# NOC-OI/ship-track-estimators

Hardware: AMD Instinct MI355X
Metric: UKF+URTSS track-steps/sec (dim=4, 500-step tracks) (higher is better)
Workload: dtype f64

## Files before the change

### ship-track-estimators_amd/csrc/ste_kernels.hip

```cpp
#include <hip/hip_runtime.h>

#include <algorithm>
#include <cstddef>
#include <cstdint>
#include <cstdio>
#include <cstring>
#include <type_traits>
#include <vector>

#include "../../include/ste.h"
#include "ste_err.h"
#include "ste_ukf.h"

namespace ste {

__shared__ int g_sched_word[2];
__device__ __forceinline__ int sched_k0() { return *(volatile int*)&g_sched_word[0]; }

template <bool kWarm>
__device__ __forceinline__ int sigma_fan(const double (&x)[4], const double (&P)[4][4], double scale,
                                         double (&sig)[9][4], EigBasis& basis);

__device__ __forceinline__ int sigma_fan(const double (&x)[4], const double (&P)[4][4], double scale,
                                         double (&sig)[9][4]) {
// ... 519 lines not shown
__device__ __forceinline__ int lane_update(const Mats& p, double (&x)[4], double (&P)[10], const double (&zin)[4],
                                           const double* noise, size_t nrow, size_t B, size_t t, UpdLik* lik = nullptr,
                                           const double* Rt = nullptr) {
    if (kFastUpd) {
        double z[4];
        STE_UNROLL
        for (int c = 0; c < 4; ++c) z[c] = zin[c];
        double r00 = p.R[0], r01 = p.R[1], r11 = p.R[5];
        if constexpr (kTrackR) {
            if (Rt) {
                r00 = Rt[(size_t)tix(0, 0) * B];
                r01 = Rt[(size_t)tix(0, 1) * B];
                r11 = Rt[(size_t)tix(1, 1) * B];
            }
        }
        int st = 0;
        if (kRobust) st = robust_rescale_sel2(p, x, P, z, r00, r01, r11);
        if (noise) {
            STE_UNROLL
            for (int c = 0; c < 4; ++c) z[c] += noise[(nrow * 4 + c) * B + t];
        }
        lane_update_sel2<kLik>(r00, r01, r11, x, P, z, lik);
        return st;
    } else {
        double Pf[4][4];
        STE_UNROLL
        for (int r = 0; r < 4; ++r) {
            STE_UNROLL
            for (int c = 0; c < 4; ++c) Pf[r][c] = P[tix(r, c)];
        }
        const int st = ukf_update<kLik, kTrackR>(p, x, Pf, zin, noise, nrow, B, t, lik, Rt);
        STE_UNROLL
        for (int r = 0; r < 4; ++r) {
            STE_UNROLL
            for (int c = r; c < 4; ++c) P[tix(r, c)] = Pf[r][c];
        }
        return st;
    }
}

__device__ __forceinline__ void store_hist(const KParams& p, size_t row, size_t B, size_t t, const double (&x)[4],
                                           const double (&P)[10]) {
    STE_UNROLL
    for (int c = 0; c < 4; ++c) st_stream(&p.fwd_mean[(row * 4 + c) * B + t], x[c]);
    store_cov_p(p.fwd_cov, (p.flags & STE_FLAG_PACKED_COV) != 0, row, B, t, P);
}

enum { kLikOff = 0, kLikHist = 1, kLikOnly = 2 };
struct LikParams {
    double* loglik;
    int32_t* dof;
    int32_t* nupd;
    double* nis;
};

template <bool kGains, bool kFastUpd, bool kRobust, bool kSched, int kLik = kLikOff, bool kTrackNoise = false>
__device__ __forceinline__ void forward_tile_l1(const KParams& p, const size_t t, const LikParams* lk = nullptr,
                                                const NoiseParams* nz = nullptr) {
    static_assert(kLik != kLikOnly || (!kGains && !kSched), "the likelihood-only pass writes no histories and no work rows");
    const size_t B = (size_t)p.ld;
    if (t >= (size_t)p.B) return;
    const bool cont = (p.flags & kFlagContinue) != 0;
    const int ns = (p.nsteps ? p.nsteps[t] - p.k0 : p.Nmax);
    if (cont && ns <= 0) return;

    double x[4], P[10];
    STE_UNROLL
    for (int c = 0; c < 4; ++c) x[c] = p.x0[c * B + t];
    if (cont && (p.flags & STE_FLAG_PACKED_COV)) {
        load_cov_p(p.P0, true, 0, B, t, P);
    } else {
        double Pf[4][4];
        if (p.flags & STE_FLAG_SHARED_P0) {
            STE_UNROLL
            for (int r = 0; r < 4; ++r) {
                STE_UNROLL
                for (int c = 0; c < 4; ++c) Pf[r][c] = p.P0[r * 4 + c];
            }
        } else {
            load_mat(p.P0, 0, B, t, Pf);
        }
        STE_UNROLL
        for (int r = 0; r < 4; ++r) {
            STE_UNROLL
            for (int c = r; c < 4; ++c) P[tix(r, c)] = 0.5 * (Pf[r][c] + Pf[c][r]);
        }
    }
    if (kLik != kLikOnly) store_hist(p, 0, B, t, x, P);

    int st = cont ? (__hip_atomic_load(&p.status[t], __ATOMIC_RELAXED, __HIP_MEMORY_SCOPE_AGENT) & ~STE_STATUS_NAN) : 0;
    const bool initial_update = !(p.flags & STE_FLAG_NO_INITIAL_UPDATE);
    const bool noise_mode = p.noise_pred || p.noise_upd || p.noise_rts;
    bool flagged = false;
    double* first_bad = (kGains && p.rts_work) ? p.first_bad + t : nullptr;
    if (first_bad) {
        if (cont)
            flagged = __hip_atomic_load(first_bad, __ATOMIC_RELAXED, __HIP_MEMORY_SCOPE_AGENT) != kNeverBad;
        else
            *first_bad = kNeverBad;
    }
    TrigReg tk;
    trig_reg_init(tk);
    double Qv[10];
    STE_UNROLL
    for (int r = 0; r < 4; ++r) {
        STE_UNROLL
        for (int c = r; c < 4; ++c) Qv[tix(r, c)] = in_vgpr(p.m.Q[r * 4 + c]);
    }
    const double* Rt = nullptr;
    if constexpr (kTrackNoise) {
        if (nz->Q) {
            STE_UNROLL
            for (int e = 0; e < 10; ++e) Qv[e] = nz->Q[(size_t)e * B + t];
        }
        if (nz->R) Rt = nz->R + t;
    }
    double V[4][4];
    if (kGains && initial_update && ns > 0) {
        double xc[4], Pc[10];
        STE_UNROLL
        for (int c = 0; c < 4; ++c) xc[c] = x[c];
        STE_UNROLL
        for (int e = 0; e < 10; ++e) Pc[e] = P[e];
        st |= lane_predict<true, kSched>(p.m, xc, Pc, V, false, p.dt[t], p.sog_rate[t], p.cog_rate[t], nullptr, p.noise_rts, 0, B, t,
                                         p.rts_work, true, noise_mode, flagged, first_bad, tk, Qv);
    }
    double lik_sum = 0.0;
    int lik_dof = 0, lik_nupd = 0;
    if (initial_update) {
        double z0[4];
        load_vec(p.z, 0, B, t, z0);
        if constexpr (kLik != kLikOff) {
            UpdLik u;
            st |= lane_update<kFastUpd, kRobust, true, kTrackNoise>(p.m, x, P, z0, p.noise_upd, 0, B, t, &u, Rt);
            lik_sum += update_loglik(u);
            lik_dof += u.rank;
            lik_nupd += 1;
            if (lk->nis) st_stream(&lk->nis[t], u.nis);
        } else {
            st |= lane_update<kFastUpd, kRobust, false, kTrackNoise>(p.m, x, P, z0, p.noise_upd, 0, B, t, nullptr, Rt);
        }
    } else if (kLik != kLikOff && lk->nis) {
        st_stream(&lk->nis[t], __builtin_nan(""));
    }

    double dt_n = 0.0, sr_n = 0.0, cr_n = 0.0;
    int ui_n = -1;
    if (ns > 0) {
        dt_n = p.dt[t];
        sr_n = p.sog_rate[t];
        cr_n = p.cog_rate[t];
        ui_n = p.upd_idx[t];
    }
    for (int k = 0; k < p.Nmax; ++k) {
        const bool live = k < ns;
        if (!__any(live)) break;
        if (live) {
            const double dt = dt_n, sr = sr_n, cr = cr_n;
            const int ui = ui_n;
            const bool ui_ok = ui < p.Tmax;
            const bool upd = ui >= 0 && ui_ok;
            double zk[4];
            load_vec(p.z, (size_t)(upd ? ui : 0), B, t, zk);
            {
                const size_t o = (size_t)(k + 1 < ns ? k + 1 : k) * B + t;
                dt_n = p.dt[o];
                sr_n = p.sog_rate[o];
                cr_n = p.cog_rate[o];
                ui_n = p.upd_idx[o];
            }
            double* work = (kGains && !(k == 0 && initial_update)) ? p.rts_work : nullptr;
            const bool warm = (k & (kColdEvery - 1)) != 0;
            st |= lane_predict<kGains, kSched>(p.m, x, P, V, warm, dt, sr, cr, p.noise_pred, p.noise_rts, (size_t)k, B, t, work,
                                               upd || noise_mode, noise_mode, flagged, first_bad, tk, Qv);
            if constexpr (kLik != kLikOff) {
                UpdLik u;
                u.nis = __builtin_nan("");
                if (upd) {
                    st |= lane_update<kFastUpd, kRobust, true, kTrackNoise>(p.m, x, P, zk, p.noise_upd, (size_t)k + 1, B, t, &u, Rt);
                    lik_sum += update_loglik(u);
                    lik_dof += u.rank;
                    lik_nupd += 1;
                }
                if (lk->nis) st_stream(&lk->nis[((size_t)k + 1) * B + t], u.nis);
            } else {
                if (upd) st |= lane_update<kFastUpd, kRobust, false, kTrackNoise>(p.m, x, P, zk, p.noise_upd, (size_t)k + 1, B, t, nullptr, Rt);
            }
            if (!ui_ok) st |= STE_STATUS_BAD_INDEX;
            if (kLik != kLikOnly) store_hist(p, (size_t)k + 1, B, t, x, P);
        }
    }
    double chk = 0.0;
    STE_UNROLL
    for (int c = 0; c < 4; ++c) chk += x[c] * 0.0;
    STE_UNROLL
    for (int e = 0; e < 10; ++e) chk += P[e] * 0.0;
    if (!(chk == 0.0)) st |= STE_STATUS_NAN;
    p.status[t] = st;
    if constexpr (kLik != kLikOff) {
        lk->loglik[t] = lik_sum;
        if (lk->dof) lk->dof[t] = lik_dof;
        if (lk->nupd) lk->nupd[t] = lik_nupd;
    }
}

template <bool kGains, bool kFastUpd, bool kRobust = false>
__global__ __launch_bounds__(64) __attribute__((amdgpu_waves_per_eu(1, 1))) void ukf_forward_l1(const KParams p) {
    forward_tile_l1<kGains, kFastUpd, kRobust, false>(p, (size_t)blockIdx.x * 64 + threadIdx.x);
}

template <bool kGains, bool kFastUpd, bool kRobust, int kLik>
__global__ __launch_bounds__(64) __attribute__((amdgpu_waves_per_eu(1, 1))) void ukf_forward_lik(const KParams p, const LikParams l) {
    forward_tile_l1<kGains, kFastUpd, kRobust, false, kLik>(p, (size_t)blockIdx.x * 64 + threadIdx.x, &l);
}

template <bool kGains, bool kFastUpd, bool kRobust, int kLik>
__global__ __launch_bounds__(64) __attribute__((amdgpu_waves_per_eu(1, 1))) void ukf_forward_tn(const KParams p, const LikParams l,
                                                                                                 const NoiseParams nz) {
    forward_tile_l1<kGains, kFastUpd, kRobust, false, kLik, true>(p, (size_t)blockIdx.x * 64 + threadIdx.x, &l, &nz);
}

struct SchedItem {
    int kp;
    int tile;
    int prog;
    int meta;
};
struct SchedParams {
    const KParams* kps;
    const SchedItem* items;
    int nrounds, nwaves;
    int* progress;
    int* window_done;
    int* error;
    unsigned long long timeout_ticks;
    int* started;
};

template <bool kGains, bool kFastUpd, bool kRobust>
__global__ __launch_bounds__(64) __attribute__((amdgpu_waves_per_eu(1, 1))) void ukf_forward_sched(const SchedParams sp) {
    typedef const KParams __attribute__((address_space(4))) ConstKParams;
    if (sp.started && threadIdx.x == 0) __hip_atomic_fetch_add(sp.started, 1, __ATOMIC_RELAXED, __HIP_MEMORY_SCOPE_AGENT);
    for (int r = 0; r < sp.nrounds; ++r) {
        const SchedItem* ip = sp.items + ((size_t)r * sp.nwaves + blockIdx.x);
        const int kp = __builtin_amdgcn_readfirstlane(ip->kp);
        if (kp < 0) continue;
        const int tile_word = __builtin_amdgcn_readfirstlane(ip->tile), prog = __builtin_amdgcn_readfirstlane(ip->prog);
        const int tile = tile_word & 0xffffff, publish = (tile_word >> 24) & 0xff;
        const int meta = __builtin_amdgcn_readfirstlane(ip->meta);
        const int slice = meta & 0xff;
        if (meta < 0 && (__hip_atomic_load(sp.error, __ATOMIC_RELAXED, __HIP_MEMORY_SCOPE_AGENT) != 0 ||
                         !sched_wait(sp.progress + prog, slice, sp.timeout_ticks))) {
            if (threadIdx.x == 0) __hip_atomic_store(sp.error, 1, __ATOMIC_RELAXED, __HIP_MEMORY_SCOPE_AGENT);
            return;
        }
        const KParams& p = *(const KParams*)(ConstKParams*)(uintptr_t)(sp.kps + kp);
        if (threadIdx.x == 0) *(volatile int*)&g_sched_word[0] = p.k0;
        forward_tile_l1<kGains, kFastUpd, kRobust, true>(p, (size_t)tile * 64 + threadIdx.x);
        if (meta & 0x40000000) {
            asm volatile("s_waitcnt vmcnt(0)" ::: "memory");
            __builtin_amdgcn_fence(__ATOMIC_RELEASE, "agent");
            asm volatile("s_waitcnt vmcnt(0)" ::: "memory");
            if (threadIdx.x == 0) {
                __hip_atomic_store(sp.progress + prog, publish, __ATOMIC_RELAXED, __HIP_MEMORY_SCOPE_AGENT);
                if (meta & 0x100)
                    __hip_atomic_fetch_add(sp.window_done + ((meta >> 9) & 0x1fffff), 1, __ATOMIC_RELAXED, __HIP_MEMORY_SCOPE_AGENT);
            }
        }
    }
}

__global__ __launch_bounds__(256) void sched_upload(uint4* __restrict__ dst, const uint4* __restrict__ src, size_t ncopy, size_t nzero) {
    const size_t stride = (size_t)gridDim.x * blockDim.x;
    for (size_t i = (size_t)blockIdx.x * blockDim.x + threadIdx.x; i < ncopy + nzero; i += stride)
        dst[i] = i < ncopy ? src[i] : make_uint4(0, 0, 0, 0);
}

__global__ __launch_bounds__(64) void sched_gate(const int* counter, int need, int* error, unsigned long long timeout_ticks) {
    if (!sched_wait(counter, need, timeout_ticks) && threadIdx.x == 0 && error)
        __hip_atomic_store(error, 2, __ATOMIC_RELAXED, __HIP_MEMORY_SCOPE_AGENT);
}


template <bool kTrackNoise>
__global__ __launch_bounds__(64) void urtss_backward_l1(const KParams p, const NoiseParams nz) {
    const size_t B = (size_t)p.ld;
    const size_t t = (size_t)blockIdx.x * 64 + threadIdx.x;
    if (t >= (size_t)p.B) return;
    auto track_Q = [&](int r, int c) -> double {
        if constexpr (kTrackNoise)
            return nz.Q[(size_t)tix(r, c) * B + t];
        else
            return p.m.Q[r * 4 + c];
    };
    const int ns = p.nsteps ? p.nsteps[t] : p.Nmax;
    const double* srp = p.sog_rate_rts ? p.sog_rate_rts : p.sog_rate;
    const double* crp = p.cog_rate_rts ? p.cog_rate_rts : p.cog_rate;

    double xs[4], Ps[4][4];
    load_vec(p.fwd_mean, (size_t)ns, B, t, xs);
    const bool packed = (p.flags & STE_FLAG_PACKED_COV) != 0;
    load_cov_m(p.fwd_cov, packed, (size_t)ns, B, t, Ps);
    store_vec(p.sm_mean, (size_t)ns, B, t, xs);
    store_cov_m(p.sm_cov, packed, (size_t)ns, B, t, Ps);
    store_pos(p, (size_t)ns, B, t, xs);

// ... 1004 lines not shown
```

### ship-track-estimators_amd/csrc/ste_math.h

```cpp
#pragma once
#include <hip/hip_runtime.h>

namespace ste {

constexpr double kEarthRadius = 6378.137;
constexpr double kDeg2Rad = 0.017453292519943295;
constexpr double kRad2Deg = 57.29577951308232;
constexpr double kPinvRcond = 1e-15;
constexpr int kMaxSweeps = 12;
constexpr double kRotTol2 = 4.930380657631324e-32;

#define STE_UNROLL _Pragma("unroll")

struct Mats {
    double fan_scale, w0, wi;
    double H[16], Q[16], R[16];
    double chi_alpha;
    int robust_iters;
};

__device__ __forceinline__ double floored_mod360(double a) {
    if (__builtin_expect(!(fabs(a) < 1e15), 0)) {
        double r = fmod(a, 360.0);
        if (r != 0.0) {
            if (r < 0.0) r += 360.0;
        } else {
            r = 0.0;
        }
        return r;
    }
    double q = floor(a * 2.7777777777777778e-03);
    double r = fma(-q, 360.0, a);
    if (r < 0.0) {
        q -= 1.0;
        r = fma(-q, 360.0, a);
    } else if (r >= 360.0) {
        q += 1.0;
        r = fma(-q, 360.0, a);
        if (r < 0.0) r = 360.0;
    }
    return r;
}
__device__ __forceinline__ double floored_mod(double a, double b) {
    (void)b;
    return floored_mod360(a);
}

__device__ __forceinline__ double wrap180(double y) { return floored_mod(y + 180.0, 360.0) - 180.0; }

__device__ __forceinline__ double rsqrt_fast(double x) {
    const double y = __builtin_amdgcn_rsq(x);
    const double e = fma(-(x * y), y, 1.0);
    return fma(y * e, fma(0.375, e, 0.5), y);
}


__device__ __forceinline__ void sincos_kernel(double r, double& s, double& c) {
    const double z = r * r;
    double ps = fma(z, 1.58969099521155010221e-10, -2.50507602534068634195e-08);
    ps = fma(z, ps, 2.75573137070700676789e-06);
    ps = fma(z, ps, -1.98412698298579493134e-04);
    ps = fma(z, ps, 8.33333333332248946124e-03);
    ps = fma(z, ps, -1.66666666666666324348e-01);
    s = fma(z * r, ps, r);
    double pc = fma(z, -1.13596475577881948265e-11, 2.08757232129817482790e-09);
    pc = fma(z, pc, -2.75573143513906633035e-07);
    pc = fma(z, pc, 2.48015872894767294178e-05);
    pc = fma(z, pc, -1.38888888888741095749e-03);
    pc = fma(z, pc, 4.16666666666666019037e-02);
    c = fma(z * z, pc, fma(-0.5, z, 1.0));
}

__device__ __forceinline__ void sincos_fast(double x, double& s, double& c) {
    if (__builtin_expect(!(fabs(x) < 1048576.0), 0)) {
        sincos(x, &s, &c);
        return;
    }
    const double n = rint(x * 0.63661977236758134308);
    double r = fma(-n, 1.57079632679489655800e+00, x);
    r = fma(-n, 6.12323399573676603587e-17, r);
    r = fma(-n, -1.49738490485916983405e-33, r);
    double sk, ck;
    sincos_kernel(r, sk, ck);
    const int q = (int)n;
    const double sv = (q & 1) ? ck : sk;
    const double cv = (q & 1) ? sk : ck;
    s = (q & 2) ? -sv : sv;
    c = ((q + 1) & 2) ? -cv : cv;
}

__device__ __forceinline__ double atan_small(double q) {
    const double z = q * q, w = z * z;
    double s1 = fma(w, 1.62858201153657823623e-02, 4.97687799461593236017e-02);
    s1 = fma(w, s1, 6.66107313738753120669e-02);
    s1 = fma(w, s1, 9.09088713343650656196e-02);
    s1 = fma(w, s1, 1.42857142725034663711e-01);
    s1 = fma(w, s1, 3.33333333333329318027e-01);
    double s2 = fma(w, -3.65315727442169155270e-02, -5.83357013379057348645e-02);
    s2 = fma(w, s2, -7.69187620504482999495e-02);
    s2 = fma(w, s2, -1.11111104054623557880e-01);
    s2 = fma(w, s2, -1.99999999998764832476e-01);
    return fma(-q, fma(z, s1, w * s2), q);
}

__device__ __forceinline__ double div_pos(double a, double b) {
    double r = __builtin_amdgcn_rcp(b);
    r = fma(fma(-b, r, 1.0), r, r);
    const double q = a * r;
    return fma(fma(-b, q, a), r, q);
}

__device__ __forceinline__ double div_earth_radius(double a) {
    constexpr double kInvR = 1.0 / kEarthRadius;
    const double q = a * kInvR;
    return fma(fma(-q, kEarthRadius, a), kInvR, q);
}

__device__ __forceinline__ double atan2_fast(double a, double b) {
    if (__builtin_expect(b > 1e-300 && fabs(a) <= 0.4375 * b, 1)) return atan_small(div_pos(a, b));
    return atan2(a, b);
}

__device__ __forceinline__ double asin_small(double x) {
    const double t = x * x;
    double pn = fma(t, 3.47933107596021167570e-05, 7.91534994289814532176e-04);
    pn = fma(t, pn, -4.00555345006794114027e-02);
    pn = fma(t, pn, 2.01212532134862925881e-01);
    pn = fma(t, pn, -3.25565818622400915405e-01);
    pn = fma(t, pn, 1.66666666666666657415e-01);
    pn *= t;
    double qd = fma(t, 7.70381505559019352791e-02, -6.88283971605453293030e-01);
    qd = fma(t, qd, 2.02094576023350569471e+00);
    qd = fma(t, qd, -2.40339491173441421878e+00);
    qd = fma(t, qd, 1.0);
    return fma(x, div_pos(pn, qd), x);
}

__device__ __forceinline__ void geodetic_finish(double lon_r, double lat_r, double sp, double cp, double sa, double ca,
                                                double sd, double cd, double& lon_out, double& lat_out) {
    const double a = sd * sa;
    const double sdca = sd * ca;
    const double b = fma(cp, cd, -(sp * sdca));
    const double sl = fma(sp, cd, cp * sdca);
    lon_out = (lon_r + atan2_fast(a, b)) * kRad2Deg;
    const double h2 = fma(a, a, b * b);
    const double cl = h2 * rsqrt_fast(h2);
    const double xs = fma(sl, cp, -(cl * sp));
    double lat2;
    if (__builtin_expect(fabs(xs) <= 0.5 && h2 > 1e-300 && cd > 0.0, 1)) {
        lat2 = lat_r + asin_small(xs);
    } else {
        lat2 = asin(sl);
    }
    lat_out = lat2 * kRad2Deg;
}

__device__ __forceinline__ void sincos_delta(double d, double& s, double& c) {
    if (__builtin_expect(fabs(d) <= 0.78539816339744828, 1)) {
        sincos_kernel(d, s, c);
    } else {
        sincos_fast(d, s, c);
    }
}

struct TrigLit {
    static constexpr double s1 = 1.58969099521155010221e-10, s2 = -2.50507602534068634195e-08, s3 = 2.75573137070700676789e-06,
                            s4 = -1.98412698298579493134e-04, s5 = 8.33333333332248946124e-03, s6 = -1.66666666666666324348e-01;
    static constexpr double c1 = -1.13596475577881948265e-11, c2 = 2.08757232129817482790e-09, c3 = -2.75573143513906633035e-07,
                            c4 = 2.48015872894767294178e-05, c5 = -1.38888888888741095749e-03, c6 = 4.16666666666666019037e-02;
};
struct TrigReg {
    double s1, s2, s3, s4, s5, s6, c1, c2, c3, c4, c5, c6;
};
__device__ __forceinline__ double in_vgpr(double v) {
    asm volatile("" : "+v"(v));
    return v;
}
__device__ __forceinline__ void trig_reg_init(TrigLit&) {}
__device__ __forceinline__ void trig_reg_init(TrigReg& k) {
    k.s1 = in_vgpr(TrigLit::s1);
    k.s2 = in_vgpr(TrigLit::s2);
    k.s3 = in_vgpr(TrigLit::s3);
    k.s4 = in_vgpr(TrigLit::s4);
    k.s5 = in_vgpr(TrigLit::s5);
    k.s6 = in_vgpr(TrigLit::s6);
    k.c1 = in_vgpr(TrigLit::c1);
    k.c2 = in_vgpr(TrigLit::c2);
    k.c3 = in_vgpr(TrigLit::c3);
    k.c4 = in_vgpr(TrigLit::c4);
    k.c5 = in_vgpr(TrigLit::c5);
    k.c6 = in_vgpr(TrigLit::c6);
}

template <int N, class K = TrigLit>
__device__ __forceinline__ void sincos_kernel_n(const double (&r)[N], double (&s)[N], double (&c)[N], const K& k = K()) {
#pragma clang fp contract(off)
    double z[N], ps[N], pc[N];
    STE_UNROLL
    for (int i = 0; i < N; ++i) z[i] = r[i] * r[i];
    STE_UNROLL
    for (int i = 0; i < N; ++i) ps[i] = fma(z[i], k.s1, k.s2);
    STE_UNROLL
    for (int i = 0; i < N; ++i) ps[i] = fma(z[i], ps[i], k.s3);
    STE_UNROLL
    for (int i = 0; i < N; ++i) ps[i] = fma(z[i], ps[i], k.s4);
    STE_UNROLL
    for (int i = 0; i < N; ++i) ps[i] = fma(z[i], ps[i], k.s5);
    STE_UNROLL
    for (int i = 0; i < N; ++i) ps[i] = fma(z[i], ps[i], k.s6);
    STE_UNROLL
    for (int i = 0; i < N; ++i) s[i] = fma(z[i] * r[i], ps[i], r[i]);
    STE_UNROLL
    for (int i = 0; i < N; ++i) pc[i] = fma(z[i], k.c1, k.c2);
    STE_UNROLL
    for (int i = 0; i < N; ++i) pc[i] = fma(z[i], pc[i], k.c3);
    STE_UNROLL
    for (int i = 0; i < N; ++i) pc[i] = fma(z[i], pc[i], k.c4);
    STE_UNROLL
    for (int i = 0; i < N; ++i) pc[i] = fma(z[i], pc[i], k.c5);
    STE_UNROLL
    for (int i = 0; i < N; ++i) pc[i] = fma(z[i], pc[i], k.c6);
    STE_UNROLL
    for (int i = 0; i < N; ++i) c[i] = fma(z[i] * z[i], pc[i], fma(-0.5, z[i], 1.0));
}

template <int N, class K = TrigLit>
__device__ __forceinline__ void sincos_fast_n(const double (&x)[N], double (&s)[N], double (&c)[N], bool& ok,
                                              const K& k = K()) {
#pragma clang fp contract(off)
    double n[N], r[N], sk[N], ck[N];
    double x_max = fabs(x[0]);
    STE_UNROLL
    for (int i = 1; i < N; ++i) x_max = fmax(x_max, fabs(x[i]));
    ok = ok && (x_max < 1048576.0);
    STE_UNROLL
    for (int i = 0; i < N; ++i) n[i] = rint(x[i] * 0.63661977236758134308);
    STE_UNROLL
    for (int i = 0; i < N; ++i) r[i] = fma(-n[i], 1.57079632679489655800e+00, x[i]);
    STE_UNROLL
    for (int i = 0; i < N; ++i) r[i] = fma(-n[i], 6.12323399573676603587e-17, r[i]);
    STE_UNROLL
    for (int i = 0; i < N; ++i) r[i] = fma(-n[i], -1.49738490485916983405e-33, r[i]);
    sincos_kernel_n<N, K>(r, sk, ck, k);
    STE_UNROLL
    for (int i = 0; i < N; ++i) {
        const int q = (int)n[i];
        const double sv = (q & 1) ? ck[i] : sk[i];
        const double cv = (q & 1) ? sk[i] : ck[i];
        s[i] = (q & 2) ? -sv : sv;
        c[i] = ((q + 1) & 2) ? -cv : cv;
    }
}

template <int N, class K = TrigLit>
__device__ __forceinline__ void sincos_delta_n(const double (&d)[N], double (&s)[N], double (&c)[N], bool& ok,
                                               const K& k = K()) {
#pragma clang fp contract(off)
    double d_max = fabs(d[0]);
    STE_UNROLL
    for (int i = 1; i < N; ++i) d_max = fmax(d_max, fabs(d[i]));
    ok = ok && (d_max <= 0.78539816339744828);
    sincos_kernel_n<N, K>(d, s, c, k);
}

struct GeoLit {
    static constexpr double t0 = 1.62858201153657823623e-02, t1 = 4.97687799461593236017e-02, t2 = 6.66107313738753120669e-02,
                            t3 = 9.09088713343650656196e-02, t4 = 1.42857142725034663711e-01, t5 = 3.33333333333329318027e-01,
                            u0 = -3.65315727442169155270e-02, u1 = -5.83357013379057348645e-02, u2 = -7.69187620504482999495e-02,
                            u3 = -1.11111104054623557880e-01, u4 = -1.99999999998764832476e-01;
    static constexpr double p0 = 3.47933107596021167570e-05, p1 = 7.91534994289814532176e-04, p2 = -4.00555345006794114027e-02,
                            p3 = 2.01212532134862925881e-01, p4 = -3.25565818622400915405e-01, p5 = 1.66666666666666657415e-01,
                            q0 = 7.70381505559019352791e-02, q1 = -6.88283971605453293030e-01, q2 = 2.02094576023350569471e+00,
                            q3 = -2.40339491173441421878e+00;
};
struct GeoReg {
    double t0, t1, t2, t3, t4, t5, u0, u1, u2, u3, u4;
    static constexpr double p0 = GeoLit::p0, p1 = GeoLit::p1, p2 = GeoLit::p2, p3 = GeoLit::p3, p4 = GeoLit::p4, p5 = GeoLit::p5,
                            q0 = GeoLit::q0, q1 = GeoLit::q1, q2 = GeoLit::q2, q3 = GeoLit::q3;
};
__device__ __forceinline__ void geo_reg_init(GeoLit&) {}
__device__ __forceinline__ void geo_reg_init(GeoReg& k) {
    k.t0 = in_vgpr(GeoLit::t0);
    k.t1 = in_vgpr(GeoLit::t1);
    k.t2 = in_vgpr(GeoLit::t2);
    k.t3 = in_vgpr(GeoLit::t3);
    k.t4 = in_vgpr(GeoLit::t4);
    k.t5 = in_vgpr(GeoLit::t5);
    k.u0 = in_vgpr(GeoLit::u0);
    k.u1 = in_vgpr(GeoLit::u1);
    k.u2 = in_vgpr(GeoLit::u2);
    k.u3 = in_vgpr(GeoLit::u3);
    k.u4 = in_vgpr(GeoLit::u4);
}

template <int N, class K = GeoLit>
__device__ __forceinline__ void atan_small_n(const double (&q)[N], double (&out)[N], const K& k = K()) {
#pragma clang fp contract(off)
    double z[N], w[N], s1[N], s2[N];
    STE_UNROLL
    for (int i = 0; i < N; ++i) {
        z[i] = q[i] * q[i];
        w[i] = z[i] * z[i];
    }
    STE_UNROLL
    for (int i = 0; i < N; ++i) s1[i] = fma(w[i], k.t0, k.t1);
    STE_UNROLL
    for (int i = 0; i < N; ++i) s1[i] = fma(w[i], s1[i], k.t2);
    STE_UNROLL
    for (int i = 0; i < N; ++i) s1[i] = fma(w[i], s1[i], k.t3);
    STE_UNROLL
    for (int i = 0; i < N; ++i) s1[i] = fma(w[i], s1[i], k.t4);
    STE_UNROLL
    for (int i = 0; i < N; ++i) s1[i] = fma(w[i], s1[i], k.t5);
    STE_UNROLL
    for (int i = 0; i < N; ++i) s2[i] = fma(w[i], k.u0, k.u1);
    STE_UNROLL
    for (int i = 0; i < N; ++i) s2[i] = fma(w[i], s2[i], k.u2);
    STE_UNROLL
    for (int i = 0; i < N; ++i) s2[i] = fma(w[i], s2[i], k.u3);
    STE_UNROLL
    for (int i = 0; i < N; ++i) s2[i] = fma(w[i], s2[i], k.u4);
    STE_UNROLL
    for (int i = 0; i < N; ++i) out[i] = fma(-q[i], fma(z[i], s1[i], w[i] * s2[i]), q[i]);
}

template <int N, class K = GeoLit>
__device__ __forceinline__ void asin_small_n(const double (&x)[N], double (&out)[N], const K& k = K()) {
// ... 445 lines not shown
```

### ship-track-estimators_amd/csrc/ste_smooth.h

```cpp
#pragma once
#include "ste_ukf.h"

namespace ste {

__device__ __forceinline__ bool work_row_full(const KParams& p, int k, int ui, bool always_full) {
    return always_full || (ui >= 0 && ui < p.Tmax) || (k == 0 && !(p.flags & STE_FLAG_NO_INITIAL_UPDATE));
}

struct RecurRow {
    double D2[8], xk[4], Pk[10];
    double shift[2];
};
template <bool kShift>
__device__ __forceinline__ void load_recur_row(const KParams& p, size_t k, size_t B, size_t t, bool d_rows23, RecurRow& g) {
    g.shift[0] = g.shift[1] = 0.0;
    if (kShift) {
        const double dt = p.dt[k * B + t];
        if (p.sog_rate_rts) g.shift[0] = (p.sog_rate_rts[k * B + t] - p.sog_rate[k * B + t]) * dt;
        if (p.cog_rate_rts) g.shift[1] = (p.cog_rate_rts[k * B + t] - p.cog_rate[k * B + t]) * dt;
    }
    const double* w = p.rts_work + (k * kWorkElems) * B + t;
    STE_UNROLL
    for (int e = 0; e < 4; ++e) g.D2[e] = w[(kWorkD + e) * B];
    if (d_rows23) {
        STE_UNROLL
        for (int e = 4; e < 8; ++e) g.D2[e] = w[(kWorkD + e) * B];
    }
    load_vec(p.fwd_mean, k, B, t, g.xk);
    load_cov_p(p.fwd_cov, (p.flags & STE_FLAG_PACKED_COV) != 0, k, B, t, g.Pk);
}

template <bool kShift, bool kTrackNoise = false>
__device__ __forceinline__ int smoother_step_gain(const KParams& p, int k, size_t B, size_t t, const RecurRow& cur,
                                                  const double (&xn)[4], const double (&Pn)[10], bool full, bool always_full,
                                                  bool all_eig, double kappa, double first_bad, double (&xb)[4],
                                                  double (&Pb)[10], double (&K)[4][4], const double* q4 = nullptr) {
    STE_UNROLL
    for (int c = 0; c < 4; ++c) xb[c] = xn[c];
    if (kShift) {
        xb[2] += cur.shift[0];
        xb[3] += cur.shift[1];
    }
    {
        double bv[4];
        STE_UNROLL
        for (int c = 0; c < 4; ++c) bv[c] = xb[c] - cur.xk[c];
        STE_UNROLL
        for (int r = 0; r < 4; ++r) {
            STE_UNROLL
            for (int c = r; c < 4; ++c) Pb[tix(r, c)] = fma(bv[r], bv[c], Pn[tix(r, c)]);
        }
    }
    if (full) {
        const double* w = p.rts_work + ((size_t)k * kWorkElems) * B + t;
        STE_UNROLL
        for (int c = 0; c < 4; ++c) xb[c] = w[(kWorkXb + c) * B];
        STE_UNROLL
        for (int e = 0; e < 10; ++e) Pb[e] = w[(kWorkPb + e) * B];
        if (kShift) {
            double bv[4];
            STE_UNROLL
            for (int c = 0; c < 4; ++c) bv[c] = xb[c] - cur.xk[c];
            if (p.noise_rts) {
                STE_UNROLL
                for (int c = 0; c < 4; ++c) bv[c] -= p.noise_rts[((size_t)k * 4 + c) * B + t];
            }
            const double s2 = cur.shift[0], s3 = cur.shift[1];
            Pb[tix(0, 2)] = fma(bv[0], s2, Pb[tix(0, 2)]);
            Pb[tix(1, 2)] = fma(bv[1], s2, Pb[tix(1, 2)]);
            Pb[tix(0, 3)] = fma(bv[0], s3, Pb[tix(0, 3)]);
            Pb[tix(1, 3)] = fma(bv[1], s3, Pb[tix(1, 3)]);
            Pb[tix(2, 2)] = fma(bv[2] + bv[2] + s2, s2, Pb[tix(2, 2)]);
            Pb[tix(3, 3)] = fma(bv[3] + bv[3] + s3, s3, Pb[tix(3, 3)]);
            Pb[tix(2, 3)] = fma(bv[2], s3, fma(s2, bv[3] + s3, Pb[tix(2, 3)]));
            xb[2] += s2;
            xb[3] += s3;
        }
    }
    double D[4][4];
    STE_UNROLL
    for (int r = 0; r < 4; ++r) {
        D[r][0] = cur.D2[r * 2 + 0];
        D[r][1] = cur.D2[r * 2 + 1];
        D[r][2] = kappa * cur.Pk[tix(r, 2)];
        D[r][3] = kappa * cur.Pk[tix(r, 3)];
    }
    if (!always_full) {
        double bv[4];
        STE_UNROLL
        for (int c = 0; c < 4; ++c) bv[c] = xb[c] - cur.xk[c];
        STE_UNROLL
        for (int r = 2; r < 4; ++r) {
            STE_UNROLL
            for (int c = 0; c < 2; ++c) {
                const double pm = full ? fma(-bv[c], bv[r], Pb[tix(c, r)]) : Pn[tix(c, r)];
                if constexpr (kTrackNoise)
                    D[r][c] = pm - q4[c * 2 + (r - 2)];
                else
                    D[r][c] = pm - p.m.Q[c * 4 + r];
            }
        }
    }
    if (__builtin_expect(__any((double)k >= first_bad), 0)) {
        if ((double)k >= first_bad) {
            const double* w = p.rts_work + ((size_t)k * kWorkElems) * B + t;
            STE_UNROLL
            for (int r = 0; r < 4; ++r) {
                D[r][2] = w[(kWorkD23 + r * 2 + 0) * B];
                D[r][3] = w[(kWorkD23 + r * 2 + 1) * B];
            }
        }
    }
    return smoother_gain(Pb, D, all_eig, K);

}

__device__ __forceinline__ void track_q4(const KParams& p, const NoiseParams& nz, size_t B, size_t t, double (&q4)[4]) {
    STE_UNROLL
    for (int c = 0; c < 2; ++c) {
        STE_UNROLL
        for (int r = 2; r < 4; ++r) q4[c * 2 + (r - 2)] = nz.Q ? nz.Q[(size_t)tix(c, r) * B + t] : p.m.Q[c * 4 + r];
    }
}

constexpr int kLeanK01 = kWorkD, kLeanK23 = kWorkD23;

struct LeanRow {
    double K[4][4], xb[4], Pb[10], xk[4], Pk[10];
};
__device__ __forceinline__ void load_lean_row(const KParams& p, size_t k, size_t B, size_t t, bool packed, LeanRow& g) {
    const double* w = p.rts_work + (k * kWorkElems) * B + t;
    STE_UNROLL
    for (int r = 0; r < 4; ++r) {
        g.K[r][0] = w[(kLeanK01 + 2 * r + 0) * B];
        g.K[r][1] = w[(kLeanK01 + 2 * r + 1) * B];
        g.K[r][2] = w[(kLeanK23 + 2 * r + 0) * B];
        g.K[r][3] = w[(kLeanK23 + 2 * r + 1) * B];
    }
    STE_UNROLL
    for (int c = 0; c < 4; ++c) g.xb[c] = w[(kWorkXb + c) * B];
    STE_UNROLL
    for (int e = 0; e < 10; ++e) g.Pb[e] = w[(kWorkPb + e) * B];
    load_vec(p.fwd_mean, k, B, t, g.xk);
    load_cov_p(p.fwd_cov, packed, k, B, t, g.Pk);
}

}
```

### ship-track-estimators_amd/csrc/ste_smooth.hip

```cpp
#include <hip/hip_runtime.h>

#include <cstddef>
#include <cstdint>

#include "../../include/ste.h"
#include "ste_err.h"
#include "ste_ukf.h"
#include "ste_smooth.h"
#include "ste_quad.h"

namespace ste {

template <bool kShift, bool kTrackNoise = false>
__device__ __forceinline__ void smooth_tile_l1(const KParams& p, const size_t t, const NoiseParams* nz = nullptr) {
    const size_t B = (size_t)p.ld;
    if (t >= (size_t)p.B) return;
    double q4[4] = {0.0, 0.0, 0.0, 0.0};
    if constexpr (kTrackNoise) track_q4(p, *nz, B, t, q4);
    const int ns = p.nsteps ? p.nsteps[t] : p.Nmax;
    const bool always_full = p.noise_pred || p.noise_upd || p.noise_rts;
    const bool all_eig = (p.tuning & STE_TUNING_EIG_GAINS) != 0;
    const double kappa = (p.m.wi + p.m.wi) * p.m.fan_scale;
    const double first_bad = p.first_bad[t];
    const int last_row = p.Nmax > 0 ? p.Nmax - 1 : 0;
    auto clampk = [&](int k) -> int { return min(max(k, 0), last_row); };

    double xs[4], Ps[10], xn[4], Pn[10];
    const bool packed = (p.flags & STE_FLAG_PACKED_COV) != 0;
    load_vec(p.fwd_mean, (size_t)ns, B, t, xs);
    load_cov_p(p.fwd_cov, packed, (size_t)ns, B, t, Ps);
    store_vec(p.sm_mean, (size_t)ns, B, t, xs);
    store_cov_p(p.sm_cov, packed, (size_t)ns, B, t, Ps);
    store_pos(p, (size_t)ns, B, t, xs);
    STE_UNROLL
    for (int c = 0; c < 4; ++c) xn[c] = xs[c];
    STE_UNROLL
    for (int e = 0; e < 10; ++e) Pn[e] = Ps[e];

    RecurRow nxt;
    int ui_n = -1;
    if (ns > 0) {
        load_recur_row<kShift>(p, (size_t)(ns - 1), B, t, always_full, nxt);
        ui_n = p.upd_idx[(size_t)(ns - 1) * B + t];
    }
    int st = 0;
    for (int k = p.Nmax - 1; k >= 0; --k) {
        if (!__any(k < ns)) continue;
        if (k < ns) {
            const RecurRow cur = nxt;
            const bool full = work_row_full(p, k, ui_n, always_full);
            double xb[4], Pb[10], K[4][4];
            st |= smoother_step_gain<kShift, kTrackNoise>(p, k, B, t, cur, xn, Pn, full, always_full, all_eig, kappa, first_bad, xb, Pb, K, q4);
            {
                const int kn = clampk(k - 1);
                load_recur_row<kShift>(p, (size_t)kn, B, t, always_full, nxt);
                ui_n = p.upd_idx[(size_t)kn * B + t];
            }
            double y[4];
            STE_UNROLL
            for (int c = 0; c < 4; ++c) y[c] = xs[c] - xb[c];
            y[3] = wrap180(y[3]);
            STE_UNROLL
            for (int r = 0; r < 4; ++r) {
                double acc = cur.xk[r];
                STE_UNROLL
                for (int c = 0; c < 4; ++c) acc = fma(K[r][c], y[c], acc);
                xs[r] = acc;
            }
            xs[3] = floored_mod(xs[3], 360.0);
            double dP[10];
            STE_UNROLL
            for (int e = 0; e < 10; ++e) dP[e] = Ps[e] - Pb[e];
            double KdP[4][4];
            STE_UNROLL
            for (int r = 0; r < 4; ++r) {
                STE_UNROLL
                for (int c = 0; c < 4; ++c) {
                    double acc = K[r][0] * dP[tix(0, c)];
                    STE_UNROLL
                    for (int i = 1; i < 4; ++i) acc = fma(K[r][i], dP[tix(i, c)], acc);
                    KdP[r][c] = acc;
                }
            }
            STE_UNROLL
            for (int r = 0; r < 4; ++r) {
                STE_UNROLL
                for (int c = r; c < 4; ++c) {
                    double acc = KdP[r][0] * K[c][0];
                    STE_UNROLL
                    for (int i = 1; i < 4; ++i) acc = fma(KdP[r][i], K[c][i], acc);
                    Ps[tix(r, c)] = cur.Pk[tix(r, c)] + acc;
                }
            }
            store_vec(p.sm_mean, (size_t)k, B, t, xs);
            store_cov_p(p.sm_cov, packed, (size_t)k, B, t, Ps);
            store_pos(p, (size_t)k, B, t, xs);
            STE_UNROLL
            for (int c = 0; c < 4; ++c) xn[c] = cur.xk[c];
            STE_UNROLL
            for (int e = 0; e < 10; ++e) Pn[e] = cur.Pk[e];
        }
    }
    double chk = 0.0;
    STE_UNROLL
    for (int c = 0; c < 4; ++c) chk += xs[c] * 0.0;
    STE_UNROLL
    for (int e = 0; e < 10; ++e) chk += Ps[e] * 0.0;
    if (!(chk == 0.0)) st |= STE_STATUS_NAN;
    if (st) atomicOr(&p.status[t], st);
}

template <bool kShift>
__global__ __launch_bounds__(64) void urtss_recur_l1(const KParams p) {
    smooth_tile_l1<kShift>(p, (size_t)blockIdx.x * 64 + threadIdx.x);
}
template <bool kShift>
__global__ __launch_bounds__(64) void urtss_recur_tn(const KParams p, const NoiseParams nz) {
    smooth_tile_l1<kShift, true>(p, (size_t)blockIdx.x * 64 + threadIdx.x, &nz);
}

template <bool kShift>
__global__ __launch_bounds__(64) void urtss_recur_sched(const SmoothSchedParams sp) {
    typedef const KParams __attribute__((address_space(4))) ConstKParams;
    const SmoothItem* ip = sp.items + blockIdx.x;
    const int kp = __builtin_amdgcn_readfirstlane(ip->kp), tile = __builtin_amdgcn_readfirstlane(ip->tile);
    const int prog = __builtin_amdgcn_readfirstlane(ip->prog), need = __builtin_amdgcn_readfirstlane(ip->need);
    if (__hip_atomic_load(sp.error, __ATOMIC_RELAXED, __HIP_MEMORY_SCOPE_AGENT) != 0 ||
        !sched_wait(sp.progress + prog, need, sp.timeout_ticks)) {
        if (threadIdx.x == 0) __hip_atomic_store(sp.error, 2, __ATOMIC_RELAXED, __HIP_MEMORY_SCOPE_AGENT);
        return;
    }
    const KParams& p = *(const KParams*)(ConstKParams*)(uintptr_t)(sp.kps + kp);
    smooth_tile_l1<kShift>(p, (size_t)tile * 64 + threadIdx.x);
}

template <bool kShift, bool kTrackNoise>
__global__ __launch_bounds__(64) void urtss_gains_all(const KParams p, const NoiseParams nz) {
    const size_t B = (size_t)p.ld;
    const size_t g = (size_t)blockIdx.x * 64 + threadIdx.x;
    if (g >= (size_t)p.B * (size_t)p.Nmax) return;
    const size_t t = g % (size_t)p.B;
    const int k = (int)(g / (size_t)p.B);
    const int ns = p.nsteps ? p.nsteps[t] : p.Nmax;
    if (k >= ns) return;
    const double fb_raw = p.first_bad[t];
    if (fb_raw < 0.0) return;
    const bool always_full = p.noise_pred || p.noise_upd || p.noise_rts;
    const bool all_eig = (p.tuning & STE_TUNING_EIG_GAINS) != 0;
    const double kappa = (p.m.wi + p.m.wi) * p.m.fan_scale;
    const bool packed = (p.flags & STE_FLAG_PACKED_COV) != 0;
    RecurRow cur;
    load_recur_row<kShift>(p, (size_t)k, B, t, always_full, cur);
    double xn[4], Pn[10];
    load_vec(p.fwd_mean, (size_t)k + 1, B, t, xn);
    load_cov_p(p.fwd_cov, packed, (size_t)k + 1, B, t, Pn);
    const bool full = work_row_full(p, k, p.upd_idx[(size_t)k * B + t], always_full);
    double xb[4], Pb[10], K[4][4], q4[4] = {0.0, 0.0, 0.0, 0.0};
    if constexpr (kTrackNoise) track_q4(p, nz, B, t, q4);
    const int st = smoother_step_gain<kShift, kTrackNoise>(p, k, B, t, cur, xn, Pn, full, always_full, all_eig, kappa, fb_raw, xb, Pb, K, q4);
    double* w = p.rts_work + ((size_t)k * kWorkElems) * B + t;
    STE_UNROLL
    for (int r = 0; r < 4; ++r) {
        w[(kLeanK01 + 2 * r + 0) * B] = K[r][0];
        w[(kLeanK01 + 2 * r + 1) * B] = K[r][1];
        w[(kLeanK23 + 2 * r + 0) * B] = K[r][2];
        w[(kLeanK23 + 2 * r + 1) * B] = K[r][3];
    }
    STE_UNROLL
    for (int c = 0; c < 4; ++c) w[(kWorkXb + c) * B] = xb[c];
    STE_UNROLL
    for (int e = 0; e < 10; ++e) w[(kWorkPb + e) * B] = Pb[e];
    if (st) atomicOr(&p.status[t], st);
}

__global__ __launch_bounds__(64) void urtss_recur_lean(const KParams p) {
    const size_t B = (size_t)p.ld;
    const size_t t = (size_t)blockIdx.x * 64 + threadIdx.x;
    if (t >= (size_t)p.B) return;
    const int ns = p.nsteps ? p.nsteps[t] : p.Nmax;
    const bool packed = (p.flags & STE_FLAG_PACKED_COV) != 0;
    const int last_row = p.Nmax > 0 ? p.Nmax - 1 : 0;
    {
        const double fb = p.first_bad[t];
        if (fb >= 0.0) p.first_bad[t] = -fb - 1.0;
    }
    double xs[4], Ps[10];
    load_vec(p.fwd_mean, (size_t)ns, B, t, xs);
    load_cov_p(p.fwd_cov, packed, (size_t)ns, B, t, Ps);
    store_vec(p.sm_mean, (size_t)ns, B, t, xs);
    store_cov_p(p.sm_cov, packed, (size_t)ns, B, t, Ps);
    store_pos(p, (size_t)ns, B, t, xs);
    LeanRow nxt;
    if (ns > 0) load_lean_row(p, (size_t)(ns - 1), B, t, packed, nxt);
    for (int k = p.Nmax - 1; k >= 0; --k) {
        if (!__any(k < ns)) continue;
        if (k < ns) {
            const LeanRow cur = nxt;
            load_lean_row(p, (size_t)min(max(k - 1, 0), last_row), B, t, packed, nxt);
            double y[4];
            STE_UNROLL
            for (int c = 0; c < 4; ++c) y[c] = xs[c] - cur.xb[c];
            y[3] = wrap180(y[3]);
            STE_UNROLL
            for (int r = 0; r < 4; ++r) {
                double acc = cur.xk[r];
                STE_UNROLL
                for (int c = 0; c < 4; ++c) acc = fma(cur.K[r][c], y[c], acc);
                xs[r] = acc;
            }
            xs[3] = floored_mod(xs[3], 360.0);
            double dP[10];
            STE_UNROLL
            for (int e = 0; e < 10; ++e) dP[e] = Ps[e] - cur.Pb[e];
            double KdP[4][4];
            STE_UNROLL
            for (int r = 0; r < 4; ++r) {
                STE_UNROLL
                for (int c = 0; c < 4; ++c) {
                    double acc = cur.K[r][0] * dP[tix(0, c)];
                    STE_UNROLL
                    for (int i = 1; i < 4; ++i) acc = fma(cur.K[r][i], dP[tix(i, c)], acc);
                    KdP[r][c] = acc;
                }
            }
            STE_UNROLL
// ... 210 lines not shown
```

Measured before the change: 7.939 billion.

## Prefetch next smoother row's stored xb/Pb and pin prefetched values in VGPRs

The RTS smoother loop now loads the next row's stored predicted mean/covariance (xb, Pb) and the upd_idx two steps ahead, one iteration early, so their global-memory latency overlaps the current step's gain and update arithmetic. Empty asm barriers (in_vgpr) force the prefetched values and the forward loop's prefetched dt/rates into vector registers, so the compiler cannot sink the loads back to their point of use. The cost is more live registers across the loop, which may lower occupancy or cause spills, and extra loads at the clamped tail rows.

```diff
diff --git a/ship-track-estimators_amd/csrc/ste_kernels.hip b/ship-track-estimators_amd/csrc/ste_kernels.hip
--- a/ship-track-estimators_amd/csrc/ste_kernels.hip
+++ b/ship-track-estimators_amd/csrc/ste_kernels.hip
@@ -695,6 +695,10 @@
         cr_n = p.cog_rate[t];
         ui_n = p.upd_idx[t];
     }
+    dt_n = in_vgpr(dt_n);
+    sr_n = in_vgpr(sr_n);
+    cr_n = in_vgpr(cr_n);
+    ui_n = in_vgpr(ui_n);
     for (int k = 0; k < p.Nmax; ++k) {
         const bool live = k < ns;
         if (!__any(live)) break;
diff --git a/ship-track-estimators_amd/csrc/ste_math.h b/ship-track-estimators_amd/csrc/ste_math.h
--- a/ship-track-estimators_amd/csrc/ste_math.h
+++ b/ship-track-estimators_amd/csrc/ste_math.h
@@ -173,6 +173,10 @@
     double s1, s2, s3, s4, s5, s6, c1, c2, c3, c4, c5, c6;
 };
 __device__ __forceinline__ double in_vgpr(double v) {
+    asm volatile("" : "+v"(v));
+    return v;
+}
+__device__ __forceinline__ int in_vgpr(int v) {
     asm volatile("" : "+v"(v));
     return v;
 }
diff --git a/ship-track-estimators_amd/csrc/ste_smooth.h b/ship-track-estimators_amd/csrc/ste_smooth.h
--- a/ship-track-estimators_amd/csrc/ste_smooth.h
+++ b/ship-track-estimators_amd/csrc/ste_smooth.h
@@ -30,18 +30,44 @@
     load_cov_p(p.fwd_cov, (p.flags & STE_FLAG_PACKED_COV) != 0, k, B, t, g.Pk);
 }
 
-template <bool kShift, bool kTrackNoise = false>
+template <bool kShift>
+__device__ __forceinline__ void consume_recur_row(bool d_rows23, RecurRow& g) {
+    if (kShift) {
+        g.shift[0] = in_vgpr(g.shift[0]);
+        g.shift[1] = in_vgpr(g.shift[1]);
+    }
+    STE_UNROLL
+    for (int e = 0; e < 4; ++e) g.D2[e] = in_vgpr(g.D2[e]);
+    if (d_rows23) {
+        STE_UNROLL
+        for (int e = 4; e < 8; ++e) g.D2[e] = in_vgpr(g.D2[e]);
+    }
+    STE_UNROLL
+    for (int c = 0; c < 4; ++c) g.xk[c] = in_vgpr(g.xk[c]);
+    STE_UNROLL
+    for (int e = 0; e < 10; ++e) g.Pk[e] = in_vgpr(g.Pk[e]);
+}
+
+__device__ __forceinline__ void load_stored_xb_pb(const KParams& p, size_t k, size_t B, size_t t, double (&xb)[4], double (&Pb)[10]) {
+    const double* w = p.rts_work + (k * kWorkElems) * B + t;
+    STE_UNROLL
+    for (int c = 0; c < 4; ++c) xb[c] = w[(kWorkXb + c) * B];
+    STE_UNROLL
+    for (int e = 0; e < 10; ++e) Pb[e] = w[(kWorkPb + e) * B];
+}
+
+template <bool kShift, bool kTrackNoise = false, bool kRowAhead = false>
 __device__ __forceinline__ int smoother_step_gain(const KParams& p, int k, size_t B, size_t t, const RecurRow& cur,
                                                   const double (&xn)[4], const double (&Pn)[10], bool full, bool always_full,
                                                   bool all_eig, double kappa, double first_bad, double (&xb)[4],
                                                   double (&Pb)[10], double (&K)[4][4], const double* q4 = nullptr) {
-    STE_UNROLL
-    for (int c = 0; c < 4; ++c) xb[c] = xn[c];
-    if (kShift) {
-        xb[2] += cur.shift[0];
-        xb[3] += cur.shift[1];
-    }
-    {
+    if (!kRowAhead || !full) {
+        STE_UNROLL
+        for (int c = 0; c < 4; ++c) xb[c] = xn[c];
+        if (kShift) {
+            xb[2] += cur.shift[0];
+            xb[3] += cur.shift[1];
+        }
         double bv[4];
         STE_UNROLL
         for (int c = 0; c < 4; ++c) bv[c] = xb[c] - cur.xk[c];
@@ -52,11 +78,7 @@
         }
     }
     if (full) {
-        const double* w = p.rts_work + ((size_t)k * kWorkElems) * B + t;
-        STE_UNROLL
-        for (int c = 0; c < 4; ++c) xb[c] = w[(kWorkXb + c) * B];
-        STE_UNROLL
-        for (int e = 0; e < 10; ++e) Pb[e] = w[(kWorkPb + e) * B];
+        if (!kRowAhead) load_stored_xb_pb(p, (size_t)k, B, t, xb, Pb);
         if (kShift) {
             double bv[4];
             STE_UNROLL
@@ -109,6 +131,13 @@
                 D[r][2] = w[(kWorkD23 + r * 2 + 0) * B];
                 D[r][3] = w[(kWorkD23 + r * 2 + 1) * B];
             }
+            if (kRowAhead) {
+                STE_UNROLL
+                for (int r = 0; r < 4; ++r) {
+                    D[r][2] = in_vgpr(D[r][2]);
+                    D[r][3] = in_vgpr(D[r][3]);
+                }
+            }
         }
     }
     return smoother_gain(Pb, D, all_eig, K);
diff --git a/ship-track-estimators_amd/csrc/ste_smooth.hip b/ship-track-estimators_amd/csrc/ste_smooth.hip
--- a/ship-track-estimators_amd/csrc/ste_smooth.hip
+++ b/ship-track-estimators_amd/csrc/ste_smooth.hip
@@ -38,28 +38,41 @@
     for (int e = 0; e < 10; ++e) Pn[e] = Ps[e];
 
     RecurRow nxt;
-    int ui_n = -1;
+    int ui_n = -1, ui_nn = -1;
+    double xb[4] = {0.0, 0.0, 0.0, 0.0}, Pb[10] = {0.0, 0.0, 0.0, 0.0, 0.0, 0.0, 0.0, 0.0, 0.0, 0.0};
     if (ns > 0) {
         load_recur_row<kShift>(p, (size_t)(ns - 1), B, t, always_full, nxt);
         ui_n = p.upd_idx[(size_t)(ns - 1) * B + t];
-    }
+        ui_nn = p.upd_idx[(size_t)clampk(ns - 2) * B + t];
+        if (work_row_full(p, ns - 1, ui_n, always_full)) load_stored_xb_pb(p, (size_t)(ns - 1), B, t, xb, Pb);
+    }
+    consume_recur_row<kShift>(always_full, nxt);
+    ui_n = in_vgpr(ui_n);
+    ui_nn = in_vgpr(ui_nn);
+    STE_UNROLL
+    for (int c = 0; c < 4; ++c) xb[c] = in_vgpr(xb[c]);
+    STE_UNROLL
+    for (int e = 0; e < 10; ++e) Pb[e] = in_vgpr(Pb[e]);
     int st = 0;
     for (int k = p.Nmax - 1; k >= 0; --k) {
         if (!__any(k < ns)) continue;
         if (k < ns) {
             const RecurRow cur = nxt;
             const bool full = work_row_full(p, k, ui_n, always_full);
-            double xb[4], Pb[10], K[4][4];
-            st |= smoother_step_gain<kShift, kTrackNoise>(p, k, B, t, cur, xn, Pn, full, always_full, all_eig, kappa, first_bad, xb, Pb, K, q4);
-            {
-                const int kn = clampk(k - 1);
-                load_recur_row<kShift>(p, (size_t)kn, B, t, always_full, nxt);
-                ui_n = p.upd_idx[(size_t)kn * B + t];
-            }
+            double K[4][4];
+            st |= smoother_step_gain<kShift, kTrackNoise, true>(p, k, B, t, cur, xn, Pn, full, always_full, all_eig, kappa, first_bad, xb, Pb, K, q4);
             double y[4];
             STE_UNROLL
             for (int c = 0; c < 4; ++c) y[c] = xs[c] - xb[c];
             y[3] = wrap180(y[3]);
+            double dP[10];
+            STE_UNROLL
+            for (int e = 0; e < 10; ++e) dP[e] = Ps[e] - Pb[e];
+            const int kn = clampk(k - 1);
+            load_recur_row<kShift>(p, (size_t)kn, B, t, always_full, nxt);
+            ui_n = ui_nn;
+            if (work_row_full(p, kn, ui_n, always_full)) load_stored_xb_pb(p, (size_t)kn, B, t, xb, Pb);
+            ui_nn = p.upd_idx[(size_t)clampk(k - 2) * B + t];
             STE_UNROLL
             for (int r = 0; r < 4; ++r) {
                 double acc = cur.xk[r];
@@ -68,9 +81,6 @@
                 xs[r] = acc;
             }
             xs[3] = floored_mod(xs[3], 360.0);
-            double dP[10];
-            STE_UNROLL
-            for (int e = 0; e < 10; ++e) dP[e] = Ps[e] - Pb[e];
             double KdP[4][4];
             STE_UNROLL
             for (int r = 0; r < 4; ++r) {
```

Result: faster. 8.052 billion (median of 6 runs) (+1.4%).
